# zyj0021200/simpleImageCaptionZoo

Hardware: AMD Instinct MI355X
Metric: captions/sec (SCST step), BUTDDetection COCO14-size vocab (higher is better)
Workload: dtype f32

## Files before the change

include/icz.h:

```cpp
#ifndef ICZ_H_
#define ICZ_H_
#include <stddef.h>
#include <stdint.h>

#ifdef __cplusplus
extern "C" {
#endif

typedef enum {
    ICZ_OK = 0,
    ICZ_ERR_INVALID = -1,
    ICZ_ERR_HIP = -2,
    ICZ_ERR_STATE = -3,
    ICZ_ERR_NOMEM = -4
} icz_status;

const char* icz_last_error(void);
const char* icz_version(void);

typedef struct icz_butd icz_butd_t;

typedef struct {
    int32_t R;
    int32_t D;
// ... 306 lines not shown
int icz_gemm_big_cfg_for(int32_t layout, int32_t M, int32_t N, int32_t K, int32_t nsplit);
int icz_gemm_tn_grouped(const float* dY, int32_t ldy, int32_t M, int32_t K, int32_t ngroups, const float* const* X, const int32_t* ldx,
                        const int32_t* cols, float* const* out, const int32_t* ldo, const int32_t* rows_live, void* stream);
int icz_gemm_tn_split_pick(int32_t M, int32_t N, int32_t K);
int icz_gemm_tn_split(const float* dY, int32_t ldy, int32_t M, const float* X, int32_t ldx, int32_t N, int32_t K, float* out, int32_t ldo,
                      float* workspace, size_t workspace_floats, const int32_t* rows_live, void* stream);
int icz_gemm_route_for(int32_t layout, int32_t M, int32_t N, int32_t nseg, const int32_t* K, int32_t nsplit);
int icz_gemm_split_for(int32_t layout, int32_t M, int32_t N, int32_t nseg, const int32_t* K, size_t workspace_floats);
int icz_gemm_tn_grouped_fits(int32_t M, int32_t K, int32_t ngroups, const int32_t* cols);
int icz_test_side_branch(int32_t fail_at, int32_t inline_branch, float* out2, void* stream);
int icz_test_embed_grad(const int64_t* tok, int32_t n_tok, const float* demb, int32_t ns, int64_t slab_stride, const float* emb, float scale,
                        int32_t E, float* dE, int32_t V, int32_t relu, const int32_t* rows_live, int32_t route, void* stream);
int icz_embed_grad_route_for(int32_t n_tok, int32_t E, size_t* lds_bytes_out);
int icz_test_weight_norm(int32_t multi, int32_t count, const float* const* v, const float* const* g, float* const* w, float* const* norm,
                         const int32_t* rows, const int32_t* cols, void* stream);
int icz_test_weight_norm_bwd(int32_t multi, int32_t count, const float* const* dw, const int32_t* lddw, const float* const* v, const float* const* g,
                             const float* const* norm, float* const* dv, float* const* dg, const int32_t* rows, const int32_t* cols, void* stream);
int icz_test_transpose(int32_t count, const float* const* src, const int32_t* ld, const int32_t* rows, const int32_t* cols, float* const* dst,
                       void* stream);
int icz_test_colsum(int32_t multi, int32_t count, const float* const* X, const int32_t* K, const int32_t* N, const int32_t* ldx, float* const* out,
                    float* const* out2, void* stream);
int icz_test_timesum(const float* X, int32_t T, int64_t BN, float* out, void* stream);
int icz_test_rowgroup_sum(const float* X, int32_t n_img, int32_t G, int64_t N, float* out, void* stream);
int icz_beam_rowtopk_route_for(int32_t V, int32_t ldl, int32_t base_aligned);
int icz_test_beam_rowtopk(int32_t route, const float* logits, int32_t n_img, int32_t k, int32_t V, int32_t ldl, int32_t step, const int32_t* n_act,
                          const float* run, int32_t compact, const int32_t* seqs_in, int32_t L, int32_t ngram, int32_t groups, float* cand_val,
                          int32_t* cand_idx, void* stream);
typedef struct {
    const float* logits;
    int32_t* n_act;
    float* run;
    const int32_t* seqs_in;
    int32_t* seqs_out;
    int32_t* src_row;
    int64_t* it_next;
    float* best_score;
    int32_t* best_len;
    int32_t* best_seq;
    int32_t* has_complete;
    int32_t* n_live;
    int32_t* hyp_seq;
    float* hyp_score;
    int32_t* hyp_len;
    int32_t* hyp_cnt;
    float* cand_val;
    int32_t* cand_idx;
// ... 20 lines not shown
```

simpleimagecaptionzoo_amd/_lib.py:

```python
import ctypes as C
import os

_HERE = os.path.dirname(os.path.abspath(__file__))
LIB_PATH = os.path.join(_HERE, "libicz.so")


class IczError(RuntimeError):
    pass


GRAD_READY_CB = C.CFUNCTYPE(None, C.c_void_p, C.c_int32)


class ButdDims(C.Structure):
    _fields_ = [(n, C.c_int32) for n in ("R", "D", "H", "E", "A", "V", "max_rows", "max_len")]


BUTD_PARAM_FIELDS = (
    "embed_weight",
    "td_w_ih", "td_w_hh", "td_b_ih", "td_b_hh",
    "lm_w_ih", "lm_w_hh", "lm_b_ih", "lm_b_hh",
    "enc_att_v", "enc_att_g", "enc_att_b",
    "dec_att_v", "dec_att_g", "dec_att_b",
    "affine_v", "affine_g", "affine_b",
# ... 220 lines not shown
        "icz_prof_stream_rate": (C.c_int, [vp, C.c_size_t, i32, vp, C.POINTER(C.c_double)]),
        "icz_adam_clamp_multi": (C.c_int, [i32, C.POINTER(vp), C.POINTER(vp), C.POINTER(vp), C.POINTER(vp), C.POINTER(i64), f32, f32, i32, vp]),
        "icz_gemm_f32": (C.c_int, [i32, vp, i32, vp, i32, vp, vp, i32, i32, i32, i32, i32, vp, C.c_size_t, vp]),
        "icz_gemm_f32_seg": (C.c_int, [i32, i32, vp, vp, vp, vp, vp, vp, vp, i32, i32, i32, i32, i32, vp, vp, C.c_size_t, C.POINTER(i32), vp]),
        "icz_gemm_resident_pair": (C.c_int, [i32, vp, vp, vp, vp, vp, i32, i32, vp, C.c_size_t, C.POINTER(i32)] * 2 + [vp, vp]),
        "icz_gemm_workspace_floats": (C.c_size_t, [i32, i32]),
        "icz_gemm_set_big_cfg": (C.c_int, [i32]),
        "icz_gemm_big_cfg_for": (C.c_int, [i32, i32, i32, i32, i32]),
        "icz_gemm_tn_grouped": (C.c_int, [vp, i32, i32, i32, i32, vp, vp, vp, vp, vp, vp, vp]),
        "icz_gemm_tn_split_pick": (C.c_int, [i32, i32, i32]),
        "icz_gemm_tn_split": (C.c_int, [vp, i32, i32, vp, i32, i32, i32, vp, i32, vp, C.c_size_t, vp, vp]),
        "icz_gemm_route_for": (C.c_int, [i32, i32, i32, i32, vp, i32]),
        "icz_gemm_split_for": (C.c_int, [i32, i32, i32, i32, vp, C.c_size_t]),
        "icz_gemm_tn_grouped_fits": (C.c_int, [i32, i32, i32, vp]),
        "icz_test_side_branch": (C.c_int, [i32, i32, vp, vp]),
        "icz_test_embed_grad": (C.c_int, [vp, i32, vp, i32, i64, vp, f32, i32, vp, i32, i32, vp, i32, vp]),
        "icz_embed_grad_route_for": (C.c_int, [i32, i32, C.POINTER(C.c_size_t)]),
        "icz_test_weight_norm": (C.c_int, [i32, i32, vp, vp, vp, vp, vp, vp, vp]),
        "icz_test_weight_norm_bwd": (C.c_int, [i32, i32, vp, vp, vp, vp, vp, vp, vp, vp, vp, vp]),
        "icz_test_transpose": (C.c_int, [i32, vp, vp, vp, vp, vp, vp]),
        "icz_test_colsum": (C.c_int, [i32, i32, vp, vp, vp, vp, vp, vp, vp]),
        "icz_test_timesum": (C.c_int, [vp, i32, i64, vp, vp]),
        "icz_test_rowgroup_sum": (C.c_int, [vp, i32, i32, i64, vp, vp]),
        "icz_beam_rowtopk_route_for": (C.c_int, [i32, i32, i32]),
        "icz_test_beam_rowtopk": (C.c_int, [i32, vp, i32, i32, i32, i32, i32, vp, vp, i32, vp, i32, i32, i32, vp, vp, vp]),
        "icz_test_beam_step": (C.c_int, [i32, C.POINTER(BeamStepState), i32, i32, i32, i32, i32, i32, i32, i32, i32, f32, vp]),
        "icz_test_beam_finalize": (C.c_int, [i32, i32, i32, i32, i32, i32, i32, f32, i32] + [vp] * 15),
    }
    for name, (res, args) in sig.items():
        try:
            fn = getattr(L, name)
        except AttributeError as e:
            raise IczError("libicz.so lacks symbol %s (stale build?)" % name) from e
        fn.restype, fn.argtypes = res, args
    _lib = L
    return L


def check(status):
    if status != 0:
        raise IczError("libicz status %d: %s" % (status, lib().icz_last_error().decode()))


def ptr(t):
    return None if t is None else C.c_void_p(t.data_ptr())

# ... 5 lines not shown
```

simpleimagecaptionzoo_amd/butd.py:

```python
import ctypes as C

import torch

from . import _lib
from ._lib import BUTD_PARAM_KEYS, ButdDims, ButdParams, Rng, check, lib, ptr, stream_ptr
from .handle import GraphDecoderHandle
from .regions import RegionSets


def make_rng(seed=0, uniforms=None, emb_mask=None, att_mask=None, out_mask=None):
    r = Rng()
    r.seed = int(seed) & 0xFFFFFFFFFFFFFFFF
    keep = []
    for name, t, dt in (("uniforms", uniforms, torch.float32), ("emb_mask", emb_mask, torch.uint8),
                        ("att_mask", att_mask, torch.uint8), ("out_mask", out_mask, torch.uint8)):
        if t is not None:
            if t.dtype != dt or not t.is_cuda or not t.is_contiguous():
                raise _lib.IczError("%s must be a contiguous %s CUDA tensor" % (name, dt))
            setattr(r, name, t.data_ptr())
            keep.append(t)
    r._keep = keep
    return r


# ... 158 lines not shown
    check(lib().icz_test_weight_norm_bwd(int(multi), len(jobs), _ptrs(c[0]), _i32s(c[1]), _ptrs(c[2]), _ptrs(c[3]), _ptrs(c[4]), _ptrs(c[5]),
                                         _ptrs(c[6]), _i32s(c[7]), _i32s(c[8]), stream_ptr()))


def transpose_multi(jobs):
    c = list(zip(*jobs)) if jobs else [()] * 5
    check(lib().icz_test_transpose(len(jobs), _ptrs(c[0]), _i32s(c[1]), _i32s(c[2]), _i32s(c[3]), _ptrs(c[4]), stream_ptr()))


def colsum(jobs, multi=True):
    c = list(zip(*jobs)) if jobs else [()] * 6
    check(lib().icz_test_colsum(int(multi), len(jobs), _ptrs(c[0]), _i32s(c[1]), _i32s(c[2]), _i32s(c[3]), _ptrs(c[4]), _ptrs(c[5]),
                                stream_ptr()))


def timesum(X, T, BN, out):
    check(lib().icz_test_timesum(ptr(X), int(T), int(BN), ptr(out), stream_ptr()))


def rowgroup_sum(X, n_img, G, N, out):
    check(lib().icz_test_rowgroup_sum(ptr(X), int(n_img), int(G), int(N), ptr(out), stream_ptr()))


def adam_clamp_step(p, g, m, v, n, lr, clip, step):
    check(lib().icz_adam_clamp_step(ptr(p), ptr(g), ptr(m), ptr(v), int(n), float(lr), float(clip), int(step), stream_ptr()))


def adam_clamp_multi(tensors, lr, clip, step):
    c = list(zip(*tensors)) if tensors else [()] * 5
    numel = (C.c_int64 * len(tensors))(*[int(n) for n in c[4]])
    check(lib().icz_adam_clamp_multi(len(tensors), _ptrs(c[0]), _ptrs(c[1]), _ptrs(c[2]), _ptrs(c[3]), numel, float(lr), float(clip), int(step),
                                     stream_ptr()))


def gemm_resident_pair(As_a, Bs_a, As_b, Bs_b, slabs_a=None, slabs_b=None, live=None):
    ta, tb = _seg_tables("nt", As_a, Bs_a), _seg_tables("nt", As_b, Bs_b)
    bufs = []
    for (n, _, _, _, _, kk, M, N), buf, As in ((ta, slabs_a, As_a), (tb, slabs_b, As_b)):
        if M is None:
            raise _lib.IczError("gemm_resident_pair: a problem without segments")
        if buf is None:
            buf = torch.empty(max(sum(kk) // 256, 1) * M * N, device=As[0].device, dtype=torch.float32)
        bufs.append(buf)
    na, nb = C.c_int32(0), C.c_int32(0)
    args = []
    for (n, ap, lda, bp, ldb, kk, M, N), buf, used in ((ta, bufs[0], na), (tb, bufs[1], nb)):
# ... 61 lines not shown
```

simpleimagecaptionzoo_amd/csrc/butd.hip:

```cpp
#include <vector>

#include "butd_impl.h"

namespace icz {

int Butd::init(const icz_butd_dims& d, int r_max) {
    dims = d;
    ICZ_REQUIRE(d.R > 0 && d.R <= r_max, "butd: R=%d must be in 1..%d (36 boxes / 49 grid cells; icz_butd_create_regions: adaptive sets, up to %d)",
                d.R, r_max, ATT_MAX_R);
    cur_R = d.R;
    ICZ_REQUIRE(d.D % 4 == 0 && d.H % 4 == 0 && d.E % 4 == 0 && d.A % 4 == 0, "butd: D,H,E,A must be multiples of 4");
    ICZ_REQUIRE(d.V > 3 && d.max_rows > 0 && d.max_len > 0, "butd: bad V/max_rows/max_len");
    const size_t rows = d.max_rows, H = d.H, D = d.D, E = d.E, A = d.A, V = d.V, R = d.R;
    ICZ_TRY(alloc((void**)&w_enc, sizeof(float) * A * D));
    ICZ_TRY(alloc((void**)&w_dec, sizeof(float) * A * H));
    ICZ_TRY(alloc((void**)&w_aff, sizeof(float) * A));
    const size_t Vp = pad_vocab(d.V);
    ICZ_TRY(alloc((void**)&w_pred, sizeof(float) * Vp * H));
    ICZ_TRY(alloc((void**)&n_enc, sizeof(float) * A));
    ICZ_TRY(alloc((void**)&n_dec, sizeof(float) * A));
    ICZ_TRY(alloc((void**)&n_aff, sizeof(float) * 4));
    ICZ_TRY(alloc((void**)&n_pred, sizeof(float) * V));
    ICZ_TRY(alloc((void**)&mean, sizeof(float) * rows * D));
    ICZ_TRY(alloc((void**)&premean, sizeof(float) * rows * 4 * H));
// ... 6 lines not shown
    }
    ICZ_TRY(alloc((void**)&emb, sizeof(float) * rows * E));
    ICZ_TRY(alloc((void**)&ctx, sizeof(float) * rows * D));
    ICZ_TRY(alloc((void**)&scores, sizeof(float) * rows * R));
    ICZ_TRY(alloc((void**)&alpha, sizeof(float) * rows * R));
    ICZ_TRY(alloc((void**)&h2drop, sizeof(float) * rows * H));
    ICZ_TRY(alloc((void**)&logits, sizeof(float) * rows * Vp));
    ICZ_TRY(alloc((void**)&amax_val, sizeof(float) * rows * ARGMAX_PARTS));
    ICZ_TRY(alloc((void**)&amax_idx, sizeof(int) * rows * ARGMAX_PARTS));
    ICZ_TRY(alloc((void**)&it, sizeof(int64_t) * rows));
    ICZ_TRY(alloc_scalars(mem));
    size_t nmax = 4 * H;
    if (A > nmax) nmax = A;
    if (V > nmax) nmax = V;
    ws_floats = (size_t)TARGET_WGS * 4096 * 2 + rows * nmax;
    {
        const size_t kmax = 2 * H + (E > D ? E : D), r128 = rows < 128 ? rows : 128;
        const size_t need = (kmax / 256 + 1) * r128 * 4 * H;
        if (need > ws_floats) ws_floats = need;
    }
    ICZ_TRY(alloc((void**)&ws, sizeof(float) * ws_floats));
    ICZ_TRY(mem.synced());
    if (const char* e = getenv("ICZ_EARLY_OUT")) early_out = atoi(e) != 0;
    if (const char* e = getenv("ICZ_MERGE_SMALL")) { const int n = atoi(e); if (n >= 0 && n <= 32) merge_small = n; }
    return ICZ_OK;
}

int Butd::refresh(hipStream_t st) {
    ICZ_REQUIRE(bound, "butd: parameters not bound");
    const int A = dims.A, D = dims.D, H = dims.H, V = dims.V;
    WeightNormTable wt = {};
    int nb = 0;
    auto add = [&](const float* v, const float* g, float* w, float* norm, int rows, int cols) {
        wt.j[wt.count++] = {v, g, w, norm, rows, cols, nb};
        nb += cdiv(rows, 4);
    };
    add(P.enc_att_v, P.enc_att_g, w_enc, n_enc, A, D);
    add(P.dec_att_v, P.dec_att_g, w_dec, n_dec, A, H);
    add(P.affine_v, P.affine_g, w_aff, n_aff, 1, A);
    add(P.predict_v, P.predict_g, w_pred, n_pred, V, H);
    hipLaunchKernelGGL(weight_norm_multi_kernel, dim3(nb), dim3(256), 0, st, wt);
    ICZ_CHECK_HIP(hipGetLastError());
    fresh = true;
    wt_fresh = false;
    return ICZ_OK;
}
// ... 214 lines not shown
}

int icz_butd_bind_params(icz_butd_t* h, const icz_butd_params* p) {
    ICZ_REQUIRE(h && p, "icz_butd_bind_params: null argument");
    ICZ_TRY(check_param_table("icz_butd_bind_params", p, sizeof(*p), (1u << 16) | (1u << 17)));
    Butd* b = reinterpret_cast<Butd*>(h);
    if (b->bound && memcmp(&b->P, p, sizeof(*p)) != 0) {
        ICZ_CHECK_HIP(hipDeviceSynchronize());
        b->gc.clear();
    }
    b->P = *p;
    b->bound = true;
    b->fresh = false;
    return ICZ_OK;
}

int icz_butd_set_option(icz_butd_t* h, const char* name, int32_t value) {
    ICZ_REQUIRE(h && name, "icz_butd_set_option: null argument");
    Butd* b = reinterpret_cast<Butd*>(h);
    if (strcmp(name, "graphs") == 0) { b->use_graphs = value != 0; return ICZ_OK; }
    if (strcmp(name, "concurrent") == 0) { b->concurrent = value != 0; return ICZ_OK; }
    if (strcmp(name, "early_out") == 0) { b->early_out = value != 0; return ICZ_OK; }
    if (strcmp(name, "small_nt") == 0) { b->small_nt = value != 0; return ICZ_OK; }
    if (strcmp(name, "group_att") == 0) { b->group_att = value != 0; return ICZ_OK; }
    if (strcmp(name, "merge_small") == 0) {
        ICZ_REQUIRE(value >= 0 && value <= 32, "icz_butd_set_option: merge_small %d outside 0..32", value);
        b->merge_small = value;
        return ICZ_OK;
    }
    set_error("icz_butd_set_option: unknown option '%s'", name);
    return ICZ_ERR_INVALID;
}

int icz_butd_set_mask_sum_global(icz_butd_t* h, const float* mask_sum_global_dev, void* stream) {
    return set_norm_global("icz_butd_set_mask_sum_global", reinterpret_cast<Butd*>(h), mask_sum_global_dev, stream);
}

int icz_butd_set_grad_callback(icz_butd_t* h, icz_grad_ready_cb cb, void* user) {
    ICZ_REQUIRE(h, "null handle");
    Butd* b = reinterpret_cast<Butd*>(h);
    b->grad_cb = cb; b->grad_cb_user = user;
    return ICZ_OK;
}

int icz_butd_refresh_weights(icz_butd_t* h, void* stream) {
    ICZ_REQUIRE(h, "null handle");
// ... 47 lines not shown
```

simpleimagecaptionzoo_amd/csrc/butd_impl.h:

```cpp
#pragma once
#include <vector>
#include <stdint.h>

#include "decoder_core.h"

namespace icz {

struct StepIO {
    int rows;
    const float* feats;
    const int32_t* img_of_row;
    int rows_per_img;
    const int64_t* it;
    bool emb_ready;
    const float *h1_in, *c1_in, *h2_in, *c2_in;
    float *h1_out, *c1_out, *h2_out, *c2_out;
    float* emb_out;
    float* gates_td_out;
    float* gates_lm_out;
    float* dec_ctx_out;
    float* alpha_out;
    float* alpha_out2; int alpha2_stride;
    float* ctx_out;
    float* h2drop_out;
// ... 49 lines not shown

    int alloc(void** p, size_t bytes) { return mem.alloc(p, bytes); }
    int init(const icz_butd_dims& d, int r_max = 64);
    int refresh(hipStream_t st);
    int gemm_nt(GemmArgs& g, const float* bias, hipStream_t st);
    int prologue(const float* feats, int n_img, hipStream_t st);
    int step(const StepIO& s, hipStream_t st);
    int zero_state(int rows, int which, hipStream_t st);
    int greedy(const float* feats, int B, int max_len, int64_t* ids_out, float* alphas_out, hipStream_t st);

    int cur_R = 0, cnt_n = 0;
    const int32_t* cnt = nullptr;
    bool adaptive() const { return cnt != nullptr || cur_R > 64; }
    int check_counts(int n_img) const {
        ICZ_REQUIRE(!cnt || n_img <= cnt_n, "butd: region counts were set for %d images, the batch has %d (icz_butd_set_regions)", cnt_n, n_img);
        return ICZ_OK;
    }

    GraphCache gc{24};
    bool use_graphs = false;
    bool graphs_on() const { return use_graphs && !cnt; }
    bool concurrent = true;
    uintptr_t opt_bits() const {
        return (concurrent ? 1 : 0) + (early_out ? 2 : 0) + 4 * merge_small + (small_nt ? 256 : 0) + (group_att ? 512 : 0) + ((uintptr_t)cur_R << 16);
    }
    int greedy_impl(const float* feats, int B, int max_len, int64_t* ids_out, float* alphas_out, hipStream_t st);
    int sample_impl(const float* feats, int B, int T, int64_t* seq_out, float* logp_out, hipStream_t st);
    int greedy_chain(const float* feats, int B, int max_len, int64_t* ids_out, float* alphas_out, hipStream_t st, bool scst = false);
    int sample_chain(const float* feats, int B, int T, int64_t* seq_out, float* logp_out, hipStream_t st, int row0 = 0, int64_t* ids_out = nullptr);
    int rollouts(const float* feats, int B, int T, const icz_rng* r, int64_t* ids_out, int64_t* seq_out, float* logp_out, hipStream_t st);
    int rollouts_impl(const float* feats, int B, int T, int64_t* ids_out, int64_t* seq_out, float* logp_out, hipStream_t st);
    SideStream side;
    SideStream low;
    icz_grad_ready_cb grad_cb = nullptr; void* grad_cb_user = nullptr;
    int sample_backward_impl(const float* reward, const icz_butd_params& G, float* loss_out, float* mask_sum_out, hipStream_t st,
                             int phases = 0xF, bool fire_cb = true);
    int merge_small = 8;
    int cur_rows = 0, cur_row0 = 0;
    bool early_out = true;
    bool bptt_early_out = false;
    bool small_nt = true;
    int cur_K = 1, cur_nimg = 0;
    bool group_att = false;

    const float* seam_feats = nullptr;
    int vocab() const override { return dims.V; }
    int row_capacity() const override { return dims.max_rows; }
    bool refreshed() const override { return fresh; }
    bool compact_step() const override { return true; }
    EmbSlot emb_slot() const override { return {P.embed_weight, emb, dims.E, 1}; }
    DeviceBuffers& buffers() override { return mem; }
    int prologue(const float* feats, int n_img, int k, const int32_t* img_of_row, hipStream_t st) override;
    int step(int rows, const int64_t* it, const int32_t* img_of_row, int rows_per_img, int cur, bool slabs, LogitsView* out,
             hipStream_t st) override;
    void gather(const int32_t* src_row, int rows, int fan, hipStream_t st) override;

    TrainBuf tb;
    icz_rng rng = {};
    const float* cur_feats = nullptr;
    int ensure_train(int B, int T);
    int train_step(const float* feats, int rows, int Bs, int t, bool train, hipStream_t st, bool emb_ready = false, int* pred_nsplit = nullptr,
                   bool skip_predict = false, const int* live = nullptr, int row0 = 0);
    int sample(const float* feats, int B, int T, const icz_rng* r, int64_t* seq_out, float* logp_out, hipStream_t st);
    int sample_n(const float* feats, int B, int K, int T, const icz_rng* r, int64_t* seq_out, float* logp_out, hipStream_t st);
// ... 25 lines not shown
```

simpleimagecaptionzoo_amd/csrc/butd_kernels.h:

```cpp
#pragma once
#include <stdlib.h>

#include "icz_common.h"
#include "rng.h"

namespace icz {
namespace {

__global__ __launch_bounds__(256) void weight_norm_kernel(const float* __restrict__ v, const float* __restrict__ g,
                                                          float* __restrict__ w, float* __restrict__ norm,
                                                          int rows, int cols) {
    const int lane = threadIdx.x & 63;
    const int row = blockIdx.x * 4 + (threadIdx.x >> 6);
    if (row >= rows) return;
    const float* vr = v + (size_t)row * cols;
    float ss = 0.f;
    for (int c = lane * 4; c < cols; c += 256) {
        f32x4 x = *reinterpret_cast<const f32x4*>(vr + c);
        ss += x[0] * x[0] + x[1] * x[1] + x[2] * x[2] + x[3] * x[3];
    }
    ss = wave_sum(ss);
    const float nrm = sqrtf(ss);
    const float s = g[row] / nrm;
    float* wr = w + (size_t)row * cols;
// ... 1251 lines not shown
    for (int i = threadIdx.x; i < n; i += 256) s += x[i];
    s = block_sum_256(s, smf);
    if (threadIdx.x == 0) out[0] = s * scale;
}

struct LstmBwdArgs {
    const float* dh_a; int ns_a;
    int lda_a;
    const float* dh_b; int ns_b; int lda_b;
    const float* dh_c; int ns_c; int lda_c;
    const float* dhdrop;
    const float* dc_in;
    const float* gates;
    const float* c_prev;
    const float* c_cur;
    float* dgates;
    float* dc_prev;
    int rows, H;
    int rows_a, rows_b, rows_c;
    int dc_in_rows;
    const int* live;
    const int* carry_live;
};
__global__ __launch_bounds__(256) void lstm_bwd_point_kernel(LstmBwdArgs a, DropCfg dc) {
    const int row = blockIdx.y;
    const int j = blockIdx.x * 256 + threadIdx.x;
    if (j >= a.H) return;
    const int H = a.H, G = 4 * H;
    const int lflag = live_flag(a.live), cflag = live_flag(a.carry_live);
    const float* g = a.gates + (size_t)row * G + j;
    const float gi = g[0], gf = g[H], gg = g[2 * H], go = g[3 * H];
    const float cc = a.c_cur[(size_t)row * H + j];
    const float cp = a.c_prev ? a.c_prev[(size_t)row * H + j] : 0.f;
    float dhd = 0.f;
    if (a.dhdrop) dhd = a.dhdrop[(size_t)row * H + j];
    if (flag_dead(lflag)) {
        float* o = a.dgates + (size_t)row * G + j;
        o[0] = 0.f; o[H] = 0.f; o[2 * H] = 0.f; o[3 * H] = 0.f;
        return;
    }
    const bool carry = cflag != 0;
    float dh = 0.f;
    if (a.dh_a && carry && row < a.rows_a) dh += sum_slabs1(a.dh_a, a.ns_a, (size_t)a.rows_a * a.lda_a, (size_t)row * a.lda_a + j);
    if (a.dh_b && row < a.rows_b) dh += sum_slabs1(a.dh_b, a.ns_b, (size_t)a.rows_b * a.lda_b, (size_t)row * a.lda_b + j);
    if (a.dh_c && row < a.rows_c) dh += sum_slabs1(a.dh_c, a.ns_c, (size_t)a.rows_c * a.lda_c, (size_t)row * a.lda_c + j);
    if (a.dhdrop) {
        float d = dhd;
        if (dc.mode) d = dc.keep((uint64_t)row * H + j) ? d * 2.0f : 0.f;
        dh += d;
    }
    const float dcin = (a.dc_in && carry && row < a.dc_in_rows) ? a.dc_in[(size_t)row * H + j] : 0.f;
    const float tc = tanhf(cc);
    const float dcv = dcin + dh * go * (1.f - tc * tc);
    float* o = a.dgates + (size_t)row * G + j;
    o[0] = dcv * gg * gi * (1.f - gi);
    o[H] = dcv * cp * gf * (1.f - gf);
    o[2 * H] = dcv * gi * (1.f - gg * gg);
    o[3 * H] = dh * tc * go * (1.f - go);
    a.dc_prev[(size_t)row * H + j] = dcv * gf;
}


constexpr int DALPHA_COLS = 512;
template <bool AD>
__global__ __launch_bounds__(256) void att_bwd_dalpha_kernel(const float* __restrict__ dctx, int ns, int ldc, int rows,
                                                             const float* __restrict__ feats, int R, int D,
                                                             float* __restrict__ dalpha_part, const int* __restrict__ live,
                                                             const int32_t* __restrict__ img_of_row,
                                                             const int32_t* __restrict__ counts) {
    __shared__ __attribute__((aligned(16))) float sd[DALPHA_COLS];
    const int lflag = live_flag(live);
    const int row = blockIdx.x, part = blockIdx.y, nparts = gridDim.y;
    const int tid = threadIdx.x, lane = tid & 63, wave = tid >> 6;
    const int c0 = part * DALPHA_COLS;
    const size_t ss = (size_t)rows * ldc;
    constexpr int NR = 5;
    const int ca = c0 + 4 * lane, cb = ca + 256;
    const bool va = ca < D, vb = cb < D;
    const int img = img_of_row ? img_of_row[row] : row;
    const int Rc = (AD && counts) ? counts[img] : R;
    const float* frow = feats + (size_t)img * R * D;
    f32x4 xa[NR], xb[NR];
// ... 653 lines not shown
```

simpleimagecaptionzoo_amd/csrc/butd_train.hip:

```cpp
#include <math.h>

#include "butd_impl.h"
#include "ens_sample.h"

namespace icz {

__global__ void sample_init_kernel(uint8_t* unf, int* nunf, int64_t* tok, int B, int T) {
    const int i = blockIdx.x * blockDim.x + threadIdx.x;
    if (i < B) { unf[i] = 1; tok[i] = 1; }
    if (i < T) nunf[i] = 0;
}

int Butd::ensure_train(int B, int T) {
    if (tb.B >= B && tb.T >= T) return ICZ_OK;
    ICZ_REQUIRE(B <= 2 * dims.max_rows, "butd: batch %d exceeds capacity %d", B, dims.max_rows);
    ICZ_REQUIRE(T <= XE_MAX_T, "butd: %d steps exceed the limit of %d", T, XE_MAX_T);
    if (tb.B > B) B = tb.B;
    if (tb.T > T) T = tb.T;
    if (dims.max_len > T) T = dims.max_len;
    if (!mem.training.empty()) {
        ICZ_TRY(mem.release_training(&gc));
        tb = TrainBuf();
        drop_loss_buffers();
    }
// ... 443 lines not shown
    ICZ_TRY(c.predict.fork(st));
    {
        GemmArgs g = gemm_args({{tb.logit, w_pred, Vp, H, Vp}}, TB, H, tb.dH2d, H);
        g.rows_live = c.rl;
        ICZ_TRY(gemm_finished(GEMM_NN, g, split_backward(STEP_WGS), nullptr, ws, ws_floats, st, "butd"));
    }
    ICZ_TRY(c.predict.start());
    hipStream_t const sb = c.predict.st();
    ICZ_TRY(wgrad(tb.logit, Vp, Vp, tb.h2d, H, H, TB, tb.dWp, H, sb, c.rl));
    (void)launch_colsum(tb.logit, TB, V, Vp, c.G.predict_b, sb);
    hipLaunchKernelGGL(weight_norm_bwd_kernel, dim3(cdiv(V, 4)), dim3(256), 0, sb, tb.dWp, H, P.predict_v, P.predict_g, n_pred,
                       c.G.predict_v, c.G.predict_g, V, H);
    ICZ_TRY(c.predict.finish());
    const bool ragged = rows_t[c.T - 1] < c.B || c.roff > 0;
    if (ragged) {
        ICZ_CHECK_HIP(hipMemsetAsync(tb.dGtd, 0, sizeof(float) * (size_t)TB * 4 * H, st));
        ICZ_CHECK_HIP(hipMemsetAsync(tb.dGlm, 0, sizeof(float) * (size_t)TB * 4 * H, st));
        ICZ_CHECK_HIP(hipMemsetAsync(tb.dDec, 0, sizeof(float) * (size_t)TB * A, st));
        ICZ_CHECK_HIP(hipMemsetAsync(tb.dS, 0, sizeof(float) * (size_t)TB * R, st));
    }
    return ICZ_OK;
}

int Butd::bptt_loop(BpttCall& c) {
    const int B = c.B, T = c.T, Bs = c.Bs, roff = c.roff;
    const int H = dims.H, D = dims.D, E = dims.E, A = dims.A, R = cur_R;
    const bool ad = adaptive();
    const size_t sH = (size_t)Bs * H;
    const float* const feats = cur_feats;
    const int32_t* const imgk = c.imgk;
    hipStream_t const st = c.st;
    int cur = 0;
    int ns1 = 1, ns2 = 1, ns3 = 1, ns4 = 1;
    int bnext = 0;
    for (int t = T - 1; t >= 0; --t) {
        const int bt = rows_t[t];
        const size_t slot = (size_t)t * Bs + roff;
        const int* const live = (bptt_early_out && early_out && t > 0) ? nunf + (t - 1) : nullptr;
        const int* const carry_live = (bptt_early_out && early_out && t + 1 < T) ? nunf + t : nullptr;
        DropCfg d_out = make_drop(d_seed, cur_train, rng.out_mask, (size_t)B * H, RNG_OUT, t);
        DropCfg d_att = make_drop(d_seed, cur_train, rng.att_mask, (size_t)B * R * A, RNG_ATT, t);
        DropCfg d_off = {0, nullptr, nullptr, 0, 0};
        {
            LstmBwdArgs a = {};
            a.dh_a = bnext ? tb.X[2] : nullptr; a.ns_a = ns3; a.lda_a = H; a.rows_a = bnext;
            a.dhdrop = tb.dH2d + slot * H;
            a.dc_in = bnext ? tb.dc2[cur] : nullptr; a.dc_in_rows = bnext;
            a.gates = tb.glm + slot * 4 * H;
            a.c_prev = tb.c2 + slot * H; a.c_cur = tb.c2 + slot * H + sH;
            a.dgates = tb.dGlm + slot * 4 * H; a.dc_prev = tb.dc2[cur ^ 1];
            a.rows = bt; a.H = H; a.live = live; a.carry_live = carry_live;
            hipLaunchKernelGGL(lstm_bwd_point_kernel, dim3(cdiv(H, 256), bt), dim3(256), 0, st, a, d_out);
        }
        const bool rdg = wt_lm_ih && wt_fresh && bt > 32 && bt <= 64 && gemm_slab_floats(bt, D + H, 4 * H / 256) <= tb.xfloats &&
                         gemm_slab_floats(bt, H, 2 * (4 * H / 256)) <= tb.xfloats;
        const bool tdg = small_nt && wt_lm_ih && wt_fresh && bt <= 32;
        const GemmLayout lay = (rdg || tdg) ? GEMM_NT : GEMM_NN;
        const float* const dglm = tb.dGlm + slot * 4 * H;
        const float* const dgtd = tb.dGtd + slot * 4 * H;
        auto wseg = [&](const float* dg, const float* w_t, const float* w, int ldw) -> GemmSeg {
            return lay == GEMM_NT ? GemmSeg{dg, w_t, 4 * H, 4 * H, 4 * H} : GemmSeg{dg, w, 4 * H, ldw, 4 * H};
        };
        auto dgrad = [&](GemmArgs g, float* slab, int* ns) -> int {
            if (!rdg) return gemm_auto(lay, g, slab, tb.xfloats, ns, st);
            *ns = gemm_resident_x3_nsplit(g);
            return gemm_slabs(GEMM_NT, g, *ns, slab, tb.xfloats, st, "butd");
        };
        ICZ_TRY(dgrad(gemm_args({wseg(dglm, wt_lm_ih, P.lm_w_ih, D + H)}, bt, D + H, tb.X[0], D + H, live), tb.X[0], &ns1));
        {
            const int dparts = cdiv(D, DALPHA_COLS);
            hipLaunchKernelGGL(ad ? att_bwd_dalpha_kernel<true> : att_bwd_dalpha_kernel<false>, dim3(bt, dparts), dim3(256), 0, st, tb.X[0], ns1, D + H, bt,
                               feats, R, D, tb.dalpha, live, imgk, cnt);
            AttBwdDdecArgs da = {enc_ctx, tb.dec + slot * A, w_aff, tb.alpha + slot * R, tb.dalpha, tb.dDec + slot * A, tb.dS + slot * R, R, A, dparts, live, imgk, cnt};
            hipLaunchKernelGGL(ad ? att_bwd_ddec_kernel<true> : att_bwd_ddec_kernel<false>, dim3(bt, cdiv(A, 256)), dim3(256), 0, st, da, d_att);
            GemmArgs g = gemm_args({{tb.dDec + slot * A, w_dec, A, H, A}}, bt, H, tb.X[1], H, live);
            ICZ_TRY(gemm_auto(GEMM_NN, g, tb.X[1], tb.xfloats, &ns2, st));
        }
        {
            LstmBwdArgs a = {};
            a.dh_a = bnext ? tb.X[3] : nullptr; a.ns_a = ns4; a.lda_a = H; a.rows_a = bnext;
            a.dh_b = tb.X[0] + D; a.ns_b = ns1; a.lda_b = D + H; a.rows_b = bt;
            a.dh_c = tb.X[1]; a.ns_c = ns2; a.lda_c = H; a.rows_c = bt;
            a.dc_in = bnext ? tb.dc1[cur] : nullptr; a.dc_in_rows = bnext;
            a.gates = tb.gtd + slot * 4 * H;
            a.c_prev = tb.c1 + slot * H; a.c_cur = tb.c1 + slot * H + sH;
            a.dgates = tb.dGtd + slot * 4 * H; a.dc_prev = tb.dc1[cur ^ 1];
            a.rows = bt; a.H = H; a.live = live; a.carry_live = carry_live;
            hipLaunchKernelGGL(lstm_bwd_point_kernel, dim3(cdiv(H, 256), bt), dim3(256), 0, st, a, d_off);
        }
        if (t > 0) {
            const GemmArgs g3 = gemm_args({wseg(dglm, wt_lm_hh, P.lm_w_hh, H), wseg(dgtd, wt_td_ih_h2, P.td_w_ih, H + D + E)}, bt, H, tb.X[2], H, live);
            const GemmArgs g4 = gemm_args({wseg(dgtd, wt_td_hh, P.td_w_hh, H)}, bt, H, tb.X[3], H, live);
            if (rdg) {
                ns3 = gemm_resident_x3_nsplit(g3); ns4 = gemm_resident_x3_nsplit(g4);
                ICZ_REQUIRE(gemm_slab_floats(bt, H, ns3) <= tb.xfloats, "butd: slab buffer too small for the dgrad slabs");
                ICZ_TRY(gemm_resident_x3_pair(g3, g4, st));
            } else {
                ICZ_TRY(dgrad(g3, tb.X[2], &ns3));
                ICZ_TRY(dgrad(g4, tb.X[3], &ns4));
            }
        }
        bnext = bt;
        cur ^= 1;
    }
    return ICZ_OK;
}

int Butd::bptt_embed_td_wgrad(BpttCall& c) {
    const int B = c.B, T = c.T, Bs = c.Bs, roff = c.roff, TB = c.TB, K = c.K, n_img = c.n_img;
    const int H = dims.H, D = dims.D, E = dims.E, V = dims.V, ldtd = H + D + E;
    const icz_butd_params& G = c.G;
// ... 311 lines not shown
    ICZ_CHECK_HIP(hipGetLastError());
    return ICZ_OK;
}

int icz_test_timesum(const float* X, int32_t T, int64_t BN, float* out, void* stream) {
    ICZ_REQUIRE(X && out, "icz_test_timesum: null argument");
    ICZ_REQUIRE(T >= 1 && BN >= 4 && BN % 4 == 0 && BN / 4 <= 0x7fffffff, "icz_test_timesum: T=%d, BN=%lld (whole groups of 4 floats)", T, (long long)BN);
    ICZ_REQUIRE(al16(X) && al16(out), "icz_test_timesum: X and out must be 16-byte aligned");
    hipLaunchKernelGGL(timesum_kernel, dim3(cdiv((int)(BN / 4), 256)), dim3(256), 0, (hipStream_t)stream, X, T, (size_t)BN, out);
    ICZ_CHECK_HIP(hipGetLastError());
    return ICZ_OK;
}

int icz_test_rowgroup_sum(const float* X, int32_t n_img, int32_t G, int64_t N, float* out, void* stream) {
    ICZ_REQUIRE(X && out, "icz_test_rowgroup_sum: null argument");
    ICZ_REQUIRE(n_img >= 1 && G >= 1 && N >= 4 && N % 4 == 0 && n_img * N / 4 <= 0x7fffffff,
                "icz_test_rowgroup_sum: n_img=%d, G=%d, N=%lld (whole groups of 4 floats)", n_img, G, (long long)N);
    ICZ_REQUIRE(al16(X) && al16(out), "icz_test_rowgroup_sum: X and out must be 16-byte aligned");
    hipLaunchKernelGGL(rowgroup_sum_kernel, dim3(cdiv((int)((size_t)n_img * N / 4), 256)), dim3(256), 0, (hipStream_t)stream, X, n_img, G, (size_t)N, out);
    ICZ_CHECK_HIP(hipGetLastError());
    return ICZ_OK;
}

}
```

Baseline: 11830.

## Fuse the dDec x W_dec GEMM into the LSTM backward pointwise kernel

In the BPTT loop, the small GEMM that turns dDec into the attention-path contribution to dh1 is folded into the LSTM backward pointwise kernel. The fused kernel computes 16x16 output tiles with MFMA, splits K across waves, reduces the partials in LDS and then applies the gate math. This removes one kernel launch and the slab write and read per timestep. In exchange, each tile is reduced serially inside one block, with fewer blocks in flight. The path is on by default when rows<=64 and H and A meet the alignment constraints, and an env/option toggle plus a test entry point are added.

```diff
diff --git a/include/icz.h b/include/icz.h
--- a/include/icz.h
+++ b/include/icz.h
@@ -352,6 +352,10 @@
                     float* const* out2, void* stream);
 int icz_test_timesum(const float* X, int32_t T, int64_t BN, float* out, void* stream);
 int icz_test_rowgroup_sum(const float* X, int32_t n_img, int32_t G, int64_t N, float* out, void* stream);
+int icz_test_bptt_dh1_step(int32_t route, int32_t rows, int32_t H, int32_t A, const float* ddec, const float* w_dec, const float* carry,
+                           int32_t ns_carry, int32_t rows_carry, const float* x1, int32_t ns_x1, int32_t ld_x1, const float* dc_in,
+                           const float* gates, const float* c_prev, const float* c_cur, float* dgates, float* dc_prev, const int32_t* live,
+                           const int32_t* carry_live, float* x2_slabs, size_t x2_floats, int32_t* nsplit_out, int32_t* route_out, void* stream);
 int icz_beam_rowtopk_route_for(int32_t V, int32_t ldl, int32_t base_aligned);
 int icz_test_beam_rowtopk(int32_t route, const float* logits, int32_t n_img, int32_t k, int32_t V, int32_t ldl, int32_t step, const int32_t* n_act,
                           const float* run, int32_t compact, const int32_t* seqs_in, int32_t L, int32_t ngram, int32_t groups, float* cand_val,
diff --git a/simpleimagecaptionzoo_amd/_lib.py b/simpleimagecaptionzoo_amd/_lib.py
--- a/simpleimagecaptionzoo_amd/_lib.py
+++ b/simpleimagecaptionzoo_amd/_lib.py
@@ -266,6 +266,7 @@
         "icz_test_colsum": (C.c_int, [i32, i32, vp, vp, vp, vp, vp, vp, vp]),
         "icz_test_timesum": (C.c_int, [vp, i32, i64, vp, vp]),
         "icz_test_rowgroup_sum": (C.c_int, [vp, i32, i32, i64, vp, vp]),
+        "icz_test_bptt_dh1_step": (C.c_int, [i32, i32, i32, i32, vp, vp, vp, i32, i32, vp, i32, i32] + [vp] * 9 + [C.c_size_t, C.POINTER(i32), C.POINTER(i32), vp]),
         "icz_beam_rowtopk_route_for": (C.c_int, [i32, i32, i32]),
         "icz_test_beam_rowtopk": (C.c_int, [i32, vp, i32, i32, i32, i32, i32, vp, vp, i32, vp, i32, i32, i32, vp, vp, vp]),
         "icz_test_beam_step": (C.c_int, [i32, C.POINTER(BeamStepState), i32, i32, i32, i32, i32, i32, i32, i32, i32, f32, vp]),
diff --git a/simpleimagecaptionzoo_amd/butd.py b/simpleimagecaptionzoo_amd/butd.py
--- a/simpleimagecaptionzoo_amd/butd.py
+++ b/simpleimagecaptionzoo_amd/butd.py
@@ -204,6 +204,16 @@
     check(lib().icz_test_rowgroup_sum(ptr(X), int(n_img), int(G), int(N), ptr(out), stream_ptr()))
 
 
+def bptt_dh1_step(route, rows, H, A, ddec, w_dec, x1, ns_x1, ld_x1, gates, c_cur, dgates, dc_prev, carry=None, ns_carry=0, rows_carry=0,
+                  dc_in=None, c_prev=None, live=None, carry_live=None, x2_slabs=None):
+    ns, taken = C.c_int32(0), C.c_int32(-1)
+    check(lib().icz_test_bptt_dh1_step(int(route), int(rows), int(H), int(A), ptr(ddec), ptr(w_dec), ptr(carry), int(ns_carry), int(rows_carry),
+                                       ptr(x1), int(ns_x1), int(ld_x1), ptr(dc_in), ptr(gates), ptr(c_prev), ptr(c_cur), ptr(dgates), ptr(dc_prev),
+                                       ptr(live), ptr(carry_live), ptr(x2_slabs), 0 if x2_slabs is None else x2_slabs.numel(), C.byref(ns),
+                                       C.byref(taken), stream_ptr()))
+    return int(ns.value), int(taken.value)
+
+
 def adam_clamp_step(p, g, m, v, n, lr, clip, step):
     check(lib().icz_adam_clamp_step(ptr(p), ptr(g), ptr(m), ptr(v), int(n), float(lr), float(clip), int(step), stream_ptr()))
 
diff --git a/simpleimagecaptionzoo_amd/csrc/butd.hip b/simpleimagecaptionzoo_amd/csrc/butd.hip
--- a/simpleimagecaptionzoo_amd/csrc/butd.hip
+++ b/simpleimagecaptionzoo_amd/csrc/butd.hip
@@ -52,6 +52,7 @@
     ICZ_TRY(alloc((void**)&ws, sizeof(float) * ws_floats));
     ICZ_TRY(mem.synced());
     if (const char* e = getenv("ICZ_EARLY_OUT")) early_out = atoi(e) != 0;
+    if (const char* e = getenv("ICZ_BPTT_FUSED_DH1")) fused_dh1 = atoi(e) != 0;
     if (const char* e = getenv("ICZ_MERGE_SMALL")) { const int n = atoi(e); if (n >= 0 && n <= 32) merge_small = n; }
     return ICZ_OK;
 }
@@ -312,6 +313,7 @@
     if (strcmp(name, "concurrent") == 0) { b->concurrent = value != 0; return ICZ_OK; }
     if (strcmp(name, "early_out") == 0) { b->early_out = value != 0; return ICZ_OK; }
     if (strcmp(name, "small_nt") == 0) { b->small_nt = value != 0; return ICZ_OK; }
+    if (strcmp(name, "fused_dh1") == 0) { b->fused_dh1 = value != 0; return ICZ_OK; }
     if (strcmp(name, "group_att") == 0) { b->group_att = value != 0; return ICZ_OK; }
     if (strcmp(name, "merge_small") == 0) {
         ICZ_REQUIRE(value >= 0 && value <= 32, "icz_butd_set_option: merge_small %d outside 0..32", value);
diff --git a/simpleimagecaptionzoo_amd/csrc/butd_impl.h b/simpleimagecaptionzoo_amd/csrc/butd_impl.h
--- a/simpleimagecaptionzoo_amd/csrc/butd_impl.h
+++ b/simpleimagecaptionzoo_amd/csrc/butd_impl.h
@@ -95,7 +95,7 @@
     bool graphs_on() const { return use_graphs && !cnt; }
     bool concurrent = true;
     uintptr_t opt_bits() const {
-        return (concurrent ? 1 : 0) + (early_out ? 2 : 0) + 4 * merge_small + (small_nt ? 256 : 0) + (group_att ? 512 : 0) + ((uintptr_t)cur_R << 16);
+        return (concurrent ? 1 : 0) + (early_out ? 2 : 0) + 4 * merge_small + (small_nt ? 256 : 0) + (group_att ? 512 : 0) + (fused_dh1 ? 1024 : 0) + ((uintptr_t)cur_R << 16);
     }
     int greedy_impl(const float* feats, int B, int max_len, int64_t* ids_out, float* alphas_out, hipStream_t st);
     int sample_impl(const float* feats, int B, int T, int64_t* seq_out, float* logp_out, hipStream_t st);
@@ -113,6 +113,7 @@
     bool early_out = true;
     bool bptt_early_out = false;
     bool small_nt = true;
+    bool fused_dh1 = true;
     int cur_K = 1, cur_nimg = 0;
     bool group_att = false;
 
diff --git a/simpleimagecaptionzoo_amd/csrc/butd_kernels.h b/simpleimagecaptionzoo_amd/csrc/butd_kernels.h
--- a/simpleimagecaptionzoo_amd/csrc/butd_kernels.h
+++ b/simpleimagecaptionzoo_amd/csrc/butd_kernels.h
@@ -1297,30 +1297,34 @@
     const int* live;
     const int* carry_live;
 };
-__global__ __launch_bounds__(256) void lstm_bwd_point_kernel(LstmBwdArgs a, DropCfg dc) {
-    const int row = blockIdx.y;
-    const int j = blockIdx.x * 256 + threadIdx.x;
-    if (j >= a.H) return;
+struct LstmBwdIn { float gi, gf, gg, go, cc, cp, dhd; };
+__device__ __forceinline__ LstmBwdIn lstm_bwd_load(const LstmBwdArgs& a, int row, int j) {
     const int H = a.H, G = 4 * H;
-    const int lflag = live_flag(a.live), cflag = live_flag(a.carry_live);
     const float* g = a.gates + (size_t)row * G + j;
-    const float gi = g[0], gf = g[H], gg = g[2 * H], go = g[3 * H];
-    const float cc = a.c_cur[(size_t)row * H + j];
-    const float cp = a.c_prev ? a.c_prev[(size_t)row * H + j] : 0.f;
-    float dhd = 0.f;
-    if (a.dhdrop) dhd = a.dhdrop[(size_t)row * H + j];
-    if (flag_dead(lflag)) {
-        float* o = a.dgates + (size_t)row * G + j;
-        o[0] = 0.f; o[H] = 0.f; o[2 * H] = 0.f; o[3 * H] = 0.f;
-        return;
-    }
-    const bool carry = cflag != 0;
+    LstmBwdIn in;
+    in.gi = g[0]; in.gf = g[H]; in.gg = g[2 * H]; in.go = g[3 * H];
+    in.cc = a.c_cur[(size_t)row * H + j];
+    in.cp = a.c_prev ? a.c_prev[(size_t)row * H + j] : 0.f;
+    in.dhd = 0.f;
+    if (a.dhdrop) in.dhd = a.dhdrop[(size_t)row * H + j];
+    return in;
+}
+__device__ __forceinline__ void lstm_bwd_dead(const LstmBwdArgs& a, int row, int j) {
+    const int H = a.H;
+    float* o = a.dgates + (size_t)row * 4 * H + j;
+    o[0] = 0.f; o[H] = 0.f; o[2 * H] = 0.f; o[3 * H] = 0.f;
+}
+__device__ __forceinline__ float lstm_bwd_dh_ab(const LstmBwdArgs& a, int row, int j, bool carry) {
     float dh = 0.f;
     if (a.dh_a && carry && row < a.rows_a) dh += sum_slabs1(a.dh_a, a.ns_a, (size_t)a.rows_a * a.lda_a, (size_t)row * a.lda_a + j);
     if (a.dh_b && row < a.rows_b) dh += sum_slabs1(a.dh_b, a.ns_b, (size_t)a.rows_b * a.lda_b, (size_t)row * a.lda_b + j);
-    if (a.dh_c && row < a.rows_c) dh += sum_slabs1(a.dh_c, a.ns_c, (size_t)a.rows_c * a.lda_c, (size_t)row * a.lda_c + j);
+    return dh;
+}
+__device__ __forceinline__ void lstm_bwd_finish(const LstmBwdArgs& a, const DropCfg& dc, int row, int j, const LstmBwdIn& in, float dh, bool carry) {
+    const int H = a.H, G = 4 * H;
+    const float gi = in.gi, gf = in.gf, gg = in.gg, go = in.go, cc = in.cc, cp = in.cp;
     if (a.dhdrop) {
-        float d = dhd;
+        float d = in.dhd;
         if (dc.mode) d = dc.keep((uint64_t)row * H + j) ? d * 2.0f : 0.f;
         dh += d;
     }
@@ -1333,6 +1337,100 @@
     o[2 * H] = dcv * gi * (1.f - gg * gg);
     o[3 * H] = dh * tc * go * (1.f - go);
     a.dc_prev[(size_t)row * H + j] = dcv * gf;
+}
+__global__ __launch_bounds__(256) void lstm_bwd_point_kernel(LstmBwdArgs a, DropCfg dc) {
+    const int row = blockIdx.y;
+    const int j = blockIdx.x * 256 + threadIdx.x;
+    if (j >= a.H) return;
+    const int lflag = live_flag(a.live), cflag = live_flag(a.carry_live);
+    const LstmBwdIn in = lstm_bwd_load(a, row, j);
+    if (flag_dead(lflag)) {
+        lstm_bwd_dead(a, row, j);
+        return;
+    }
+    const bool carry = cflag != 0;
+    float dh = lstm_bwd_dh_ab(a, row, j, carry);
+    if (a.dh_c && row < a.rows_c) dh += sum_slabs1(a.dh_c, a.ns_c, (size_t)a.rows_c * a.lda_c, (size_t)row * a.lda_c + j);
+    lstm_bwd_finish(a, dc, row, j, in, dh, carry);
+}
+
+struct Dh1FusedArgs {
+    LstmBwdArgs p;
+    const float* ddec;
+    const float* w_dec;
+    int A;
+    int ns, cps;
+};
+constexpr int DH1_TILE = 16, DH1_MAX_SPLIT = 32;
+inline bool lstm_bwd_dh1_fused_takes(int rows, int H, int A) {
+    return rows >= 1 && rows <= 64 && H >= DH1_TILE && H % DH1_TILE == 0 && A >= 64 && A % 64 == 0;
+}
+inline int lstm_bwd_dh1_stage_k(int A) { return A % 128 == 0 ? 128 : 64; }
+
+template <int BKC>
+__global__ __launch_bounds__(256) void lstm_bwd_dh1_fused_kernel(Dh1FusedArgs f) {
+    constexpr int NS = BKC / 16;
+    __shared__ float part[DH1_MAX_SPLIT][DH1_TILE * DH1_TILE];
+    const LstmBwdArgs& a = f.p;
+    const int lflag = live_flag(a.live), cflag = live_flag(a.carry_live);
+    const int tid = threadIdx.x, lane = tid & 63, wave = tid >> 6;
+    const int li = lane & 15, lq = lane >> 4;
+    const int n0 = blockIdx.x * DH1_TILE, m0 = blockIdx.y * DH1_TILE;
+    const int row = m0 + (tid >> 4), j = n0 + (tid & 15);
+    const bool valid = row < a.rows;
+    LstmBwdIn in = {};
+    if (valid) in = lstm_bwd_load(a, row, j);
+
+    const int mrow = m0 + li;
+    const float* const arow = f.ddec + (size_t)(mrow < a.rows ? mrow : a.rows - 1) * f.A + 4 * lq;
+    const float* const bcol = f.w_dec + (size_t)(4 * lq) * a.H + n0 + li;
+    const int tot = f.A / BKC;
+    f32x4 av[NS], an[NS];
+    float bv[4 * NS], bn[4 * NS];
+    auto load_stage = [&](int c, f32x4 (&x)[NS], float (&w)[4 * NS]) {
+        const int k0 = c * BKC;
+#pragma unroll
+        for (int s = 0; s < NS; ++s) x[s] = *reinterpret_cast<const f32x4*>(arow + k0 + 16 * s);
+#pragma unroll
+        for (int m = 0; m < 4 * NS; ++m) w[m] = bcol[(size_t)(k0 + 16 * (m >> 2) + (m & 3)) * a.H];
+    };
+    int z = wave, c = z * f.cps, c_end = c + f.cps < tot ? c + f.cps : tot;
+    bool have = z < f.ns;
+    if (have) load_stage(c, av, bv);
+    if (flag_dead(lflag)) {
+        if (valid) lstm_bwd_dead(a, row, j);
+        return;
+    }
+    const bool carry = cflag != 0;
+    float dh = 0.f;
+    if (valid) dh = lstm_bwd_dh_ab(a, row, j, carry);
+    f32x4 acc = {0.f, 0.f, 0.f, 0.f};
+    while (have) {
+        int z2 = z, c2 = c + 1, c_end2 = c_end;
+        if (c2 >= c_end) { z2 = z + 4; c2 = z2 * f.cps; c_end2 = c2 + f.cps < tot ? c2 + f.cps : tot; }
+        const bool more = z2 < f.ns;
+        if (more) load_stage(c2, an, bn);
+        __builtin_amdgcn_sched_barrier(0);
+#pragma unroll
+        for (int m = 0; m < 4 * NS; ++m) acc = __builtin_amdgcn_mfma_f32_16x16x4f32(av[m >> 2][m & 3], bv[m], acc, 0, 0, 0);
+        if (c + 1 >= c_end) {
+#pragma unroll
+            for (int r = 0; r < 4; ++r) part[z][(4 * lq + r) * DH1_TILE + li] = acc[r];
+            acc = (f32x4){0.f, 0.f, 0.f, 0.f};
+        }
+#pragma unroll
+        for (int s = 0; s < NS; ++s) av[s] = an[s];
+#pragma unroll
+        for (int m = 0; m < 4 * NS; ++m) bv[m] = bn[m];
+        z = z2; c = c2; c_end = c_end2; have = more;
+    }
+    __syncthreads();
+    if (!valid) return;
+    float x2 = 0.f;
+    for (int s = 0; s < f.ns; ++s) x2 += part[s][tid];
+    dh += x2;
+    const DropCfg off = {};
+    lstm_bwd_finish(a, off, row, j, in, dh, carry);
 }
 
 
diff --git a/simpleimagecaptionzoo_amd/csrc/butd_train.hip b/simpleimagecaptionzoo_amd/csrc/butd_train.hip
--- a/simpleimagecaptionzoo_amd/csrc/butd_train.hip
+++ b/simpleimagecaptionzoo_amd/csrc/butd_train.hip
@@ -489,6 +489,24 @@
     return ICZ_OK;
 }
 
+static int dh1_split(int rows, int H, int A) {
+    const GemmArgs g = gemm_args({{nullptr, nullptr, A, H, A}}, rows, H, nullptr, H);
+    return gemm_split(GEMM_NN, g, split_backward(Butd::STEP_WGS), 0);
+}
+static int launch_dh1_fused(const LstmBwdArgs& p, const float* ddec, const float* w_dec, int A, hipStream_t st) {
+    ICZ_REQUIRE(lstm_bwd_dh1_fused_takes(p.rows, p.H, A), "butd: the fused d h1 step does not take rows=%d, H=%d, A=%d", p.rows, p.H, A);
+    const int bkc = lstm_bwd_dh1_stage_k(A), tot = A / bkc, ns = dh1_split(p.rows, p.H, A);
+    ICZ_REQUIRE(ns >= 1 && ns <= DH1_MAX_SPLIT && ns <= tot, "butd: the fused d h1 step cannot mirror %d K ranges over %d stages", ns, tot);
+    const int cps = cdiv(tot, ns);
+    ICZ_REQUIRE(cdiv(tot, cps) == ns, "butd: the fused d h1 step cannot mirror %d K ranges over %d stages", ns, tot);
+    const Dh1FusedArgs f = {p, ddec, w_dec, A, ns, cps};
+    const dim3 grid(p.H / DH1_TILE, cdiv(p.rows, DH1_TILE));
+    if (bkc == 128) hipLaunchKernelGGL(lstm_bwd_dh1_fused_kernel<128>, grid, dim3(256), 0, st, f);
+    else hipLaunchKernelGGL(lstm_bwd_dh1_fused_kernel<64>, grid, dim3(256), 0, st, f);
+    ICZ_CHECK_HIP(hipGetLastError());
+    return ICZ_OK;
+}
+
 int Butd::bptt_loop(BpttCall& c) {
     const int B = c.B, T = c.T, Bs = c.Bs, roff = c.roff;
     const int H = dims.H, D = dims.D, E = dims.E, A = dims.A, R = cur_R;
@@ -523,6 +541,7 @@
                          gemm_slab_floats(bt, H, 2 * (4 * H / 256)) <= tb.xfloats;
         const bool tdg = small_nt && wt_lm_ih && wt_fresh && bt <= 32;
         const GemmLayout lay = (rdg || tdg) ? GEMM_NT : GEMM_NN;
+        const bool fdh = fused_dh1 && lstm_bwd_dh1_fused_takes(bt, H, A);
         const float* const dglm = tb.dGlm + slot * 4 * H;
         const float* const dgtd = tb.dGtd + slot * 4 * H;
         auto wseg = [&](const float* dg, const float* w_t, const float* w, int ldw) -> GemmSeg {
@@ -540,20 +559,23 @@
                                feats, R, D, tb.dalpha, live, imgk, cnt);
             AttBwdDdecArgs da = {enc_ctx, tb.dec + slot * A, w_aff, tb.alpha + slot * R, tb.dalpha, tb.dDec + slot * A, tb.dS + slot * R, R, A, dparts, live, imgk, cnt};
             hipLaunchKernelGGL(ad ? att_bwd_ddec_kernel<true> : att_bwd_ddec_kernel<false>, dim3(bt, cdiv(A, 256)), dim3(256), 0, st, da, d_att);
-            GemmArgs g = gemm_args({{tb.dDec + slot * A, w_dec, A, H, A}}, bt, H, tb.X[1], H, live);
-            ICZ_TRY(gemm_auto(GEMM_NN, g, tb.X[1], tb.xfloats, &ns2, st));
+            if (!fdh) {
+                GemmArgs g = gemm_args({{tb.dDec + slot * A, w_dec, A, H, A}}, bt, H, tb.X[1], H, live);
+                ICZ_TRY(gemm_auto(GEMM_NN, g, tb.X[1], tb.xfloats, &ns2, st));
+            }
         }
         {
             LstmBwdArgs a = {};
             a.dh_a = bnext ? tb.X[3] : nullptr; a.ns_a = ns4; a.lda_a = H; a.rows_a = bnext;
             a.dh_b = tb.X[0] + D; a.ns_b = ns1; a.lda_b = D + H; a.rows_b = bt;
-            a.dh_c = tb.X[1]; a.ns_c = ns2; a.lda_c = H; a.rows_c = bt;
+            if (!fdh) { a.dh_c = tb.X[1]; a.ns_c = ns2; a.lda_c = H; a.rows_c = bt; }
             a.dc_in = bnext ? tb.dc1[cur] : nullptr; a.dc_in_rows = bnext;
             a.gates = tb.gtd + slot * 4 * H;
             a.c_prev = tb.c1 + slot * H; a.c_cur = tb.c1 + slot * H + sH;
             a.dgates = tb.dGtd + slot * 4 * H; a.dc_prev = tb.dc1[cur ^ 1];
             a.rows = bt; a.H = H; a.live = live; a.carry_live = carry_live;
-            hipLaunchKernelGGL(lstm_bwd_point_kernel, dim3(cdiv(H, 256), bt), dim3(256), 0, st, a, d_off);
+            if (fdh) ICZ_TRY(launch_dh1_fused(a, tb.dDec + slot * A, w_dec, A, st));
+            else hipLaunchKernelGGL(lstm_bwd_point_kernel, dim3(cdiv(H, 256), bt), dim3(256), 0, st, a, d_off);
         }
         if (t > 0) {
             const GemmArgs g3 = gemm_args({wseg(dglm, wt_lm_hh, P.lm_w_hh, H), wseg(dgtd, wt_td_ih_h2, P.td_w_ih, H + D + E)}, bt, H, tb.X[2], H, live);
@@ -911,4 +933,41 @@
     return ICZ_OK;
 }
 
-}
+int icz_test_bptt_dh1_step(int32_t route, int32_t rows, int32_t H, int32_t A, const float* ddec, const float* w_dec, const float* carry,
+                           int32_t ns_carry, int32_t rows_carry, const float* x1, int32_t ns_x1, int32_t ld_x1, const float* dc_in,
+                           const float* gates, const float* c_prev, const float* c_cur, float* dgates, float* dc_prev, const int32_t* live,
+                           const int32_t* carry_live, float* x2_slabs, size_t x2_floats, int32_t* nsplit_out, int32_t* route_out, void* stream) {
+    const char* who = "icz_test_bptt_dh1_step";
+    ICZ_REQUIRE(route >= -1 && route <= 1, "%s: route=%d (-1: as the loop picks, 0: two launches, 1: fused)", who, route);
+    ICZ_REQUIRE(rows >= 1 && rows <= 64 && H >= 4 && H % 4 == 0 && A >= 4 && A % 4 == 0, "%s: rows=%d (1..64), H=%d, A=%d (H and A in whole groups of 4)", who, rows, H, A);
+    ICZ_REQUIRE(ddec && w_dec && x1 && gates && c_cur && dgates && dc_prev, "%s: null argument", who);
+    ICZ_REQUIRE(al16(ddec) && al16(w_dec), "%s: ddec and w_dec must be 16-byte aligned", who);
+    ICZ_REQUIRE(ns_x1 >= 1 && ld_x1 >= H, "%s: ns_x1=%d, ld_x1=%d (at least H)", who, ns_x1, ld_x1);
+    ICZ_REQUIRE(!carry || (ns_carry >= 1 && rows_carry >= 1), "%s: ns_carry=%d, rows_carry=%d", who, ns_carry, rows_carry);
+    ICZ_REQUIRE(!dc_in || rows_carry >= 1, "%s: dc_in with rows_carry=%d", who, rows_carry);
+    const bool takes = lstm_bwd_dh1_fused_takes(rows, H, A);
+    ICZ_REQUIRE(route != 1 || takes, "%s: the fused kernel does not take rows=%d, H=%d, A=%d", who, rows, H, A);
+    const bool fdh = route == 1 || (route == -1 && takes);
+    const int ns = dh1_split(rows, H, A);
+    if (nsplit_out) *nsplit_out = ns;
+    if (route_out) *route_out = fdh ? 1 : 0;
+    hipStream_t const st = (hipStream_t)stream;
+    LstmBwdArgs a = {};
+    a.dh_a = carry; a.ns_a = ns_carry; a.lda_a = H; a.rows_a = rows_carry;
+    a.dh_b = x1; a.ns_b = ns_x1; a.lda_b = ld_x1; a.rows_b = rows;
+    a.dc_in = dc_in; a.dc_in_rows = rows_carry;
+    a.gates = gates; a.c_prev = c_prev; a.c_cur = c_cur; a.dgates = dgates; a.dc_prev = dc_prev;
+    a.rows = rows; a.H = H; a.live = live; a.carry_live = carry_live;
+    if (fdh) return launch_dh1_fused(a, ddec, w_dec, A, st);
+    ICZ_REQUIRE(x2_slabs && al16(x2_slabs) && gemm_slab_floats(rows, H, ns) <= x2_floats, "%s: the two-launch route needs %d slabs of rows x H floats (16-byte aligned)", who, ns);
+    GemmArgs g = gemm_args({{ddec, w_dec, A, H, A}}, rows, H, x2_slabs, H, live);
+    int ns2 = 1;
+    ICZ_TRY(gemm_slabs(GEMM_NN, g, split_backward(Butd::STEP_WGS), x2_slabs, x2_floats, &ns2, st, who));
+    a.dh_c = x2_slabs; a.ns_c = ns2; a.lda_c = H; a.rows_c = rows;
+    const DropCfg d_off = {0, nullptr, nullptr, 0, 0};
+    hipLaunchKernelGGL(lstm_bwd_point_kernel, dim3(cdiv(H, 256), rows), dim3(256), 0, st, a, d_off);
+    ICZ_CHECK_HIP(hipGetLastError());
+    return ICZ_OK;
+}
+
+}
```

After: 11990, median of 6. 1.4% higher.
